# viswavi/speech-anonymization

Measured on AMD Instinct MI355X. Metric: audio frames/sec (node), ConvAE+gender-adv train step, higher is better.
Workload: dtype bf16x3; 1 GPU; ConvAE recon0.1+sex0.9 adversarial train step (L1 recon + NLL), shape M: 32 utt/GPU x 161120 samples (T=1008 frames), Fbank x2 + norm + fwd + bwd + clip + Adam + Noam; batch_per_gpu=32, frames_per_utt=1008, parallelism=dp1

## Files before the change

### include/sa_hip.h

```cpp
#ifndef SA_HIP_H
#define SA_HIP_H
#ifdef __cplusplus
extern "C" {
#endif

#define SA_F32 0
#define SA_BF16 1
#define SA_BF16X3 2
#define SA_BF16X1F 3
#define SA_FP8 4
#define SA_F64 5
#define SA_MAX_TAPS 5
#define SA_COMM_ID_BYTES 128

typedef struct SaTaps {
  int ntaps[2];
  int off[2][SA_MAX_TAPS];
  int widx[2][SA_MAX_TAPS];
} SaTaps;

typedef struct SaConvArgs {
  const void* x;
  const void* wp;
  const float* bias;
// ... 59 lines not shown
  const float* slabs; float* dst;
  int nslab, ntaps, cin, cout, sk, sn, st, accumulate, vec, pad_;
} SaWredDesc;
typedef struct SaWredMulti { int n, pad_; SaWredDesc d[SA_WRED_MAX]; } SaWredMulti;
int sa_wgrad_reduce_multi(const SaWredMulti* m, void* stream);

int sa_conv1toC(int dtype, const float* x, const float* w, const float* bias, void* y, int B, int L,
                int flip, float* stats, const void* ep_x, const float* ep_s1, const float* ep_t1,
                const float* ep_mean, const float* ep_rstd, void* stream);
int sa_conv1toC_ntiles(int L);
int sa_convCto1(int dtype, const void* x, const float* w, const float* bias, float* y, int B, int L,
                const float* s1, const float* t1, int swish, int flip, void* stream);
int sa_wgrad1C(int dtype, const float* u, const void* v, float* slabs, int B, int L, int chunk,
               int flip, const float* s1, const float* t1, int swish, void* stream);
int sa_wgrad1C_nchunk(int L, int chunk);
int sa_sum_slabs(const float* slabs, float* dst, int nslab, int n, int accumulate, void* stream);

typedef struct SaEwArgs {
  const void* g; const void* g2; const void* x; void* out;
  const float* s1; const float* t1;
  const float* mean; const float* rstd;
  const float* c1; const float* c2; const float* c3;
  int actbwd, xp_is_act, relu_mask, bstride;
  float* stats;
  int B, L, ntiles;
} SaEwArgs;

int sa_ew_stats(int dtype, int C, const SaEwArgs* a, void* stream);
int sa_ew_apply(int dtype, int C, const SaEwArgs* a, void* stream);
int sa_ew_ntiles(int L);
// ... 141 lines not shown
                  void* stream);
int sa_fc_wreduce(const float* wpart, int G, float* grads, void* stream);

int sa_cluster_mi(const float* X, const long long* y, const long long* idx, int iters, int n, int D,
                  int ncls, int k, float* mi, void* stream);

int sa_fbank(const float* wav, int B, int N, const float* window, const void* dft,
             const void* mel, float* feats, float* tilemax, void* stream);
int sa_fbank_table_elems(int which);
int sa_fbank_ntiles(int T);
int sa_fbank_scratch_bytes(int B);
int sa_fbank_normalize(const float* feats, const float* tilemax, int B, int T, int Tp,
                       const float* lens, float top_db, int batch_max, int update, int epoch,
                       int update_until_epoch, float* state, float* scratch, float* out,
                       void* stream);

int sa_add_layernorm_fwd(const void* x, const void* r, const void* gamma, const void* beta, void* y, void* s_out,
                         float* stat, int rows, int d, float eps, void* stream);
int sa_layernorm_bwd(const void* dy, const void* s, const float* stat, const void* gamma, void* ds, int rows,
                     int d, void* stream);
int sa_ln_leaky_fwd(const void* x, const void* gamma, const void* beta, void* y, float* stat, int rows, int d,
                    float eps, float slope, void* stream);
int sa_ln_leaky_bwd(const void* dy, const void* x, const float* stat, const void* gamma, const void* beta, void* dx,
                    int rows, int d, float slope, void* stream);
int sa_asr_block0_fwd(const void* x, const void* w, const void* bias, const void* gamma, const void* beta, void* y,
                      float* stat, int B, int T, int F, int C, float eps, float slope, void* stream);
int sa_asr_block0_bwd(const void* dy, const void* x, const void* w, const void* bias, const void* gamma,
                      const void* beta, const float* stat, float* part, void* dx, int B, int T, int F, int C,
                      float slope, void* stream);
int sa_reflect_pad_fwd(const void* x, void* y, int B, int T, int F, int C, void* stream);
// ... 16 lines not shown
```

### speech-anonymization_amd/_lib.py

```python
import ctypes as C
import os

import torch

_HERE = os.path.dirname(os.path.abspath(__file__))
LIB_PATH = os.environ.get("SA_HIP_LIB") or os.path.join(_HERE, "libsa_hip.so")

F32, BF16, BF16X3, BF16X1F, FP8, F64 = 0, 1, 2, 3, 4, 5
MAX_TAPS = 5

c_fp = C.POINTER(C.c_float)
vp = C.c_void_p


class SaTaps(C.Structure):
    _fields_ = [("ntaps", C.c_int * 2), ("off", (C.c_int * MAX_TAPS) * 2),
                ("widx", (C.c_int * MAX_TAPS) * 2)]


class SaConvArgs(C.Structure):
    _fields_ = [("x", vp), ("wp", vp), ("bias", vp), ("y", vp),
                ("s1", vp), ("t1", vp), ("s2", vp), ("t2", vp),
                ("swish", C.c_int), ("relu", C.c_int), ("stats", vp),
                ("B", C.c_int), ("Lin", C.c_int), ("Lout", C.c_int), ("ntiles", C.c_int),
# ... 67 lines not shown



class SaWredDesc(C.Structure):
    _fields_ = [("slabs", vp), ("dst", vp)] + [(k, C.c_int) for k in ("nslab", "ntaps", "cin", "cout", "sk", "sn", "st",
                                                                      "accumulate", "vec", "pad_")]


class SaWredMulti(C.Structure):
    _fields_ = [("n", C.c_int), ("pad_", C.c_int), ("d", SaWredDesc * WRED_MAX)]


SYMBOLS = [
    "sa_conv_gemm", "sa_abi_sizeof", "sa_conv_gemm_ntiles", "sa_conv_gemm_ntiles_tm", "sa_conv_gemm_set_tile_rows",
    "sa_conv_gemm_geometry", "sa_conv_gemm_set_impl", "sa_conv_gemm_route", "sa_conv_pp_set_tile_rows", "sa_pack_weights", "sa_pack_weights_multi", "sa_pack_scales_multi", "sa_wgrad", "sa_wgrad_kw", "sa_wgrad_reduce",
    "sa_conv1toC", "sa_conv1toC_ntiles", "sa_convCto1", "sa_wgrad1C", "sa_wgrad1C_nchunk",
    "sa_sum_slabs", "sa_ew_stats", "sa_ew_apply", "sa_ew_ntiles", "sa_act_stats",
    "sa_sum_partials", "sa_sum_rows_d", "sa_reduce_finalize", "sa_fin_in_fwd", "sa_fin_bn_fwd", "sa_fin_bn_eval", "sa_fin_norm_bwd", "sa_fin_bias",
    "sa_pool_fwd", "sa_pool_nseg", "sa_pool_gather", "sa_pool_fin", "sa_pool_bwd", "sa_dense", "sa_colsums",
    "sa_bn2d_bwd", "sa_dense_wgrad", "sa_log_softmax", "sa_log_softmax_bwd",
    "sa_loss_workspace_bytes", "sa_recon_loss", "sa_cls_losses", "sa_cosine_loss",
    "sa_tdnn_fwd", "sa_time_pool", "sa_leaky_affine", "sa_tdnn_bwd_input", "sa_tdnn_fold", "sa_time_pool_bwd",
    "sa_leaky_affine_bwd", "sa_cluster_mi", "sa_fbank", "sa_fbank_table_elems", "sa_fbank_ntiles", "sa_fbank_scratch_bytes", "sa_fbank_normalize",
    "sa_comm_unique_id", "sa_comm_init", "sa_comm_world", "sa_comm_allreduce", "sa_comm_allreduce_inline", "sa_comm_join", "sa_comm_ncalls",
    "sa_comm_destroy", "sa_head_fwd", "sa_head_bwd", "sa_head_max_rows",
    "sa_add_layernorm_fwd", "sa_layernorm_bwd", "sa_reflect_pad_fwd", "sa_reflect_pad_bwd", "sa_ln_leaky_fwd", "sa_ln_leaky_bwd", "sa_bias_multi", "sa_asr_block0_fwd", "sa_asr_block0_bwd", "sa_wgrad_reduce_multi", "sa_clip_grads",
    "sa_xv_tdnn_fwd_train", "sa_xv_tdnn_ntiles", "sa_xv_colsums", "sa_xv_tdnn_wgrad", "sa_xv_wgrad_reduce",
    "sa_xv_tdnn_dgrad", "sa_xv_pool_affine", "sa_xv_pool_affine_bwd",
    "sa_fc_tiles", "sa_fc_groups", "sa_fc_nparam", "sa_fc_nhead", "sa_fc_max_rows", "sa_fc_enc_fwd", "sa_fc_bn_fin",
    "sa_fc_mid_fwd", "sa_fc_head_fwd", "sa_fc_head_bwd", "sa_fc_mid_bwd", "sa_fc_bn_bwd_fin", "sa_fc_enc_bwd",
    "sa_fc_wreduce", "sa_fc_recon_fwd",
]

_lib = None


class SaHipError(RuntimeError):
    pass
# ... 60 lines not shown
```

### speech-anonymization_amd/brain.py

```python
import enum
import os
import types

import torch

from . import distributed as sdist


class Stage(enum.Enum):
    TRAIN = 1
    VALID = 2
    TEST = 3


class EpochCounter:

    def __init__(self, limit):
        self.current, self.limit = 0, int(limit)

    def __iter__(self):
        return self

    def __next__(self):
        if self.current < self.limit:
# ... 60 lines not shown

class Brain:
    GC_FREEZE_STEP = 8

    def __init__(self, modules=None, opt_class=None, hparams=None, run_opts=None, checkpointer=None):
        run_opts = dict(run_opts or {})
        self.device = torch.device(run_opts.get("device", "cuda:0" if torch.cuda.is_available() else "cpu"))
        if self.device.type == "cuda":
            torch.cuda.set_device(self.device)
        self.max_grad_norm = float(run_opts.get("max_grad_norm", 5.0))
        self.nonfinite_patience = int(run_opts.get("nonfinite_patience", 3))
        self.lazy_finite_check = bool(run_opts.get("lazy_finite_check", True))
        self.hip_graph = bool(run_opts.get("hip_graph", False)) and self.device.type == "cuda"
        self.gc_freeze = bool(run_opts.get("gc_freeze", True))
        self.fused_clip = bool(run_opts.get("fused_clip", os.environ.get("SA_FUSED_CLIP", "1") == "1"))
        self.distributed_launch = bool(run_opts.get("distributed_launch", sdist.is_distributed()))
        self.modules = torch.nn.ModuleDict(modules or {})
        self.dp_batch_sizes = run_opts.get("dp_batch_sizes", "equal")
        self.opt_class = opt_class
        self.hparams = types.SimpleNamespace(**(hparams or {}))
        self.checkpointer = checkpointer
        self.step, self.nonfinite_count, self.optimizer = 0, 0, None
        self.avg_train_loss = 0.0

    def compute_forward(self, batch, stage):
        raise NotImplementedError

    def compute_objectives(self, predictions, batch, stage):
        raise NotImplementedError

# ... 165 lines not shown
    def evaluate(self, test_set, max_key=None, min_key=None, **_):
        self.on_evaluate_start(max_key=max_key, min_key=min_key)
        self.on_stage_start(Stage.TEST, None)
        self.modules.eval()
        avg, n = 0.0, 0
        with torch.no_grad():
            for batch in test_set:
                n += 1
                avg += (float(self.evaluate_batch(batch, Stage.TEST)) - avg) / n
        self.on_stage_end(Stage.TEST, avg, None)
        return avg


class SexAnonymizationTraining(Brain):

    def features(self, wavs, wav_lens):
        feats = self.hparams.compute_features(wavs)
        current_epoch = self.hparams.epoch_counter.current
        pad = 36 if self.hparams.model_type != "fcae" else None
        return self.modules.normalize(feats, wav_lens, epoch=current_epoch, pad_multiple=pad)

    def compute_forward(self, batch, stage):
        batch = batch.to(self.device)
        wavs, wav_lens = batch.sig
        feats = self.features(wavs, wav_lens)
        return self.modules.ConvAE(feats)

    def compute_objectives(self, predictions, batch, stage):
        reconstructed_speech, sex_logits = predictions
        batch = batch.to(self.device)
        sex_label = batch.gender
        wavs, wav_lens = batch.sig
        feats = self.features(wavs, wav_lens)
        hp = self.hparams
        utility_loss = 0.0
        asr_brain = getattr(self, "asr_brain", None)
        if stage == Stage.TRAIN and hp.utility_loss_weight > 0 and asr_brain is not None:
            from . import asr
            tokens_bos, _ = batch.tokens_bos
            utility_loss = asr.utility_loss(asr_brain, hp.loss_utility, feats, reconstructed_speech,
# ... 65 lines not shown
    GRAPH_WARMUP = 3

    def _graph_key(self, batch):
        hp = self.hparams
        wavs, lens = batch.sig
        nrm = self.modules["normalize"] if "normalize" in self.modules else None
        upd = nrm is not None and hp.epoch_counter.current < getattr(nrm, "update_until_epoch", 0)
        st = self.optimizer.state if self.optimizer is not None else {}
        params = list(self.modules.ConvAE.parameters())
        tok = batch.tokens_bos[0]
        return (tuple(wavs.shape), str(wavs.dtype), hp.model_type, float(hp.recon_loss_weight),
                float(hp.sex_loss_weight), float(hp.utility_loss_weight),
                float(getattr(hp, "confusion_loss_weight", 0.0)), bool(upd),
                tuple(p.requires_grad for p in params),
                tuple(bool(st.get(p)) for p in params if not p.requires_grad),
                tuple(tok.shape), getattr(self, "asr_brain", None) is not None)

    def _step_core(self, batch):
        predictions = self.compute_forward(batch, Stage.TRAIN)
        loss = self.compute_objectives(predictions, batch, Stage.TRAIN)
        loss.backward()
        if getattr(self.hparams, "epoch_parity_schedule", False):
            self._zero_grads_of_frozen()
        self.check_gradients(loss)
        self.optimizer.step()
        return loss.detach()

    def _fit_batch_graph(self, batch):
        batch = batch.to(self.device)
        key = self._graph_key(batch)
        graphs = self.__dict__.setdefault("_graphs", {})
# ... 31 lines not shown
        ent["batch"].id = batch.id
        bad = self._poll_nonfinite()
        if bad:
            self.nonfinite_count += bad
            if self.nonfinite_count > self.nonfinite_patience:
                raise ValueError("Loss is not finite and patience is exhausted.")
        ent["graph"].replay()
        st = getattr(self, "_finite_state", None)
        if st is not None:
            st["event"].record()
            st["pending"] = True
        self.hparams.noam_annealing(self.optimizer)
        return ent["loss"]

    def fit_batch(self, batch):
        self.apply_epoch_schedule()
        if (self.hip_graph and self.hparams.gradient_accumulation == 1 and sdist.capturable()
                and self.optimizer is not None):
            return self._fit_batch_graph(batch)
        predictions = self.compute_forward(batch, Stage.TRAIN)
        loss = self.compute_objectives(predictions, batch, Stage.TRAIN)
        (loss / self.hparams.gradient_accumulation).backward()
        if self.step % self.hparams.gradient_accumulation == 0:
            if getattr(self.hparams, "epoch_parity_schedule", False):
                self._zero_grads_of_frozen()
            self.check_gradients(loss)
            self.optimizer.step()
            self.optimizer.zero_grad()
            self.hparams.noam_annealing(self.optimizer)
        return loss.detach()

    def evaluate_batch(self, batch, stage):
        with torch.no_grad():
            predictions = self.compute_forward(batch, stage=stage)
# ... 82 lines not shown
```

### speech-anonymization_amd/convae.py

```python
import functools
import os

import torch
import torch.nn as nn

from . import distributed as sdist
from . import ops
from . import _lib as L
from ._lib import SaHipError

K5 = 5
CONVT_WG_TAPS = [(1, 0), (1, 1), (0, 0), (0, 1), (-1, 0)]


class _ParamOnly(nn.Module):

    def forward(self, x):
        raise SaHipError("parameter container only; use ConvAutoencoder.forward")


class GLU(_ParamOnly):
    pass


# ... 49 lines not shown
        self.sex_classifier = TDNNSexClassifier(2)
        self.act_dtype, self.kcode = ops.PRECISIONS[precision]
        self.dec_kcode = self.kcode
        self.dgrad_kcode = ops.DGRAD_CODE[precision]
        self.cache_wgrad_operand = cache_wgrad_operand
        self.fuse_apply = True
        self.overlap_wgrad = os.environ.get("SA_OVERLAP_WGRAD", "0") == "1"
        self.pooling_noise = pooling_noise
        self.sync_bn = sync_bn
        self.fused_finalize = os.environ.get("SA_FUSED_FINALIZE", "0") == "1"
        self.fused_in_fwd = os.environ.get("SA_FUSED_IN_FWD", "0") == "1"
        self.overlap_head = os.environ.get("SA_OVERLAP_HEAD", "0") == "1"
        self.fused_head = os.environ.get("SA_FUSED_HEAD", "1") == "1"
        self.batch_bias = os.environ.get("SA_BATCH_BIAS", "1") == "1"
        self.batch_wred = os.environ.get("SA_BATCH_WRED", "1") == "1"
        self.dp_batch_sizes = None
        self.bwd_reload_bf16 = os.environ.get("SA_BWD_RELOAD_BF16", "0") == "1"
        self.store_bf16_probe = int(os.environ.get("SA_STORE_BF16_PROBE", "0"))

    def forward(self, feats):
        names, params = self._named_params()
        return _ConvAEFn.apply(self, names, feats, *params)

    def _named_params(self):
        c = self.__dict__.get("_np_cache")
        if c is None or any(o[n] is not p for o, n, p in c[2]):
            names, params, owners = [], [], []
            for mname, mod in self.named_modules():
                for pname, p in mod._parameters.items():
                    if p is not None:
# ... 602 lines not shown
            xp4 = (n4[2], n4[3])
            g, st = cg(g, pw(t + "0.weight", "conv_dgrad"), None, 128, 128, 1, 1,
                       ops.taps_conv_dgrad_s1(5, 1, 0), L4, want_stats=True, ep=bn_ep(y4, bn_n, xp4))
            da = bn_finish(g, st, y4, bn_n, L4, "sex_classifier.norm", None, 0, xp=xp4)
            side_join()
            flush_bias()
            if need_stage["sex_classifier"]:
                buckets.reduce_stage("sex_classifier")
            return da

        def decoder_bwd():
            d_rec = torch.zeros(B, T, 80, device=dev) if recon_unused else d_recon
            g_rec = d_rec.reshape(B, Ltot).contiguous().float()
            if need["decoder.8.bias"]:
                setg("decoder.8.bias", ops.sum_partials(g_rec.view(4 * B, Ltot // 4), 1, n=Ltot // 4).sum())
            if need["decoder.8.weight"]:
                G["decoder.8.weight"] = ops.wgrad1C(g_rec, y8, newg("decoder.8.weight"), flip=True,
                                                    s1=n8[2], t1=n8[3], swish=True)
            g, st = ops.conv1toC(g_rec, P["decoder.8.weight"], None, dt, flip=True, want_stats=True,
                                 ep=dict(x=y8, s1=n8[2], t1=n8[3], mean=n8[0], rstd=n8[1]))
            if model.store_bf16_probe >= 2:
                _round_first(g)
            in_decoder[0] = True
            g = in_finish(g, st, y8, n8, 32, Ltot, "decoder.6", "decoder.5.bias")
            convT_wgrad("decoder.5.weight", y7, g, 64, 32, L2)
            g, st = cg(g, pw("decoder.5.weight", "convT_dgrad"), None, 32, 64, 2, 1,
                       ops.taps_convT_dgrad(), L2, want_stats=True)
            bias_from(st, "decoder.4.bias", 64)
            conv_wgrad("decoder.4.weight", y6, g, 64, 64, 1, L2, K5, 1, 2, s1=n6[2], t1=n6[3], swish=True)
            g, st = cg(g, pw("decoder.4.weight", "conv_dgrad"), None, 64, 64, 1, 1,
                       ops.taps_conv_dgrad_s1(K5, 1, 2), L2, want_stats=True, ep=in_ep(y6, n6))
            g = in_finish(g, st, y6, n6, 64, L2, "decoder.2", "decoder.1.bias")
            convT_wgrad("decoder.1.weight", y5, g, 128, 64, L4)
            g, st = cg(g, pw("decoder.1.weight", "convT_dgrad"), None, 64, 128, 2, 1,
                       ops.taps_convT_dgrad(), L4, want_stats=True)
# ... 58 lines not shown
```

### speech-anonymization_amd/csrc/sa_fbank.hip

```cpp
#include "sa_common.h"

#define SA_NFFT 400
#define SA_HOP 160
#define SA_NBIN 201
#define SA_FK 208
#define SA_FKS 13
#define SA_BINT 7
#define SA_MELT 3
#define SA_NMEL 80
#define SA_FB_FRAMES 32

__device__ static inline void sa_split3(float v, bf16_t& h, bf16_t& m, bf16_t& l) {
  h = (bf16_t)v;
  const float r1 = v - (float)h;
  m = (bf16_t)r1;
  l = (bf16_t)(r1 - (float)m);
}

__global__ __launch_bounds__(256) void sa_fbank_kernel(const float* __restrict__ wav, int N, int T,
                                                       const float* __restrict__ window,
                                                       const bf16x8* __restrict__ dft,
                                                       const bf16x8* __restrict__ mel,
                                                       float* __restrict__ feats,
                                                       float* __restrict__ tilemax, int ntiles) {
// ... 264 lines not shown
  if (!feats || !tilemax || !lens || !state || !scratch || !out || B <= 0 || T <= 0 || Tp < T)
    return -22;
  hipStream_t st = reinterpret_cast<hipStream_t>(stream);
  float* fl = scratch;
  double* part = reinterpret_cast<double*>(scratch + ((B + 1) & ~1));
  hipLaunchKernelGGL(sa_fbank_utt_partial_kernel, dim3(SA_UTT_CHUNKS, B), dim3(256), 0, st, feats,
                     tilemax, sa_div_up(T, SA_FB_FRAMES), B, T, lens, top_db, batch_max, fl, part);
  hipLaunchKernelGGL(sa_norm_update_kernel, dim3(1), dim3(640), 0, st, part, lens, B, T, update, epoch,
                     update_until_epoch, state);
  const size_t n4 = (size_t)Tp * SA_NMEL / 4;
  hipLaunchKernelGGL(sa_norm_apply_kernel, dim3((unsigned)((n4 + 255) / 256), B), dim3(256), 0, st,
                     feats, fl, state, T, Tp, out);
  hipError_t e = hipGetLastError();
  return e == hipSuccess ? 0 : -(int)e;
}
```

### speech-anonymization_amd/csrc/sa_small.hip

```cpp
#include "sa_common.h"

#define SA_K15 15
#define SA_C32 32

template <typename T>
__global__ __launch_bounds__(256) void sa_conv1toC_kernel(const float* __restrict__ x,
                                                          const float* __restrict__ w,
                                                          const float* __restrict__ bias,
                                                          T* __restrict__ y, int L, int flip,
                                                          float* __restrict__ stats, int ntiles,
                                                          const T* __restrict__ ep_x,
                                                          const float* __restrict__ ep_s1,
                                                          const float* __restrict__ ep_t1,
                                                          const float* __restrict__ ep_mean,
                                                          const float* __restrict__ ep_rstd) {
  constexpr int VEC = Tr<T>::VEC, CH = SA_C32 / VEC, PPP = 256 / CH, TILE = 512;
  __shared__ float xs[TILE + SA_K15 - 1];
  __shared__ __attribute__((aligned(16))) float ws[SA_K15][SA_C32];
  __shared__ float red[PPP][SA_C32][2];
  const int tid = threadIdx.x, b = blockIdx.y, l0 = blockIdx.x * TILE;
  for (int i = tid; i < TILE + SA_K15 - 1; i += 256) {
    const int g = l0 + i - 7;
    xs[i] = (g >= 0 && g < L) ? x[(size_t)b * L + g] : 0.0f;
  }
// ... 261 lines not shown
                          int chunk, int flip, const float* s1, const float* t1, int swish,
                          void* stream) {
  if (!u || !v || !slabs || B <= 0 || L <= 0 || chunk <= 0 || chunk % 256) return -22;
  hipStream_t st = reinterpret_cast<hipStream_t>(stream);
  dim3 grid(sa_div_up(L, chunk), B);
  if (dtype == SA_BF16)
    hipLaunchKernelGGL(sa_wgrad1C_kernel<bf16_t>, grid, dim3(256), 0, st, u,
                       reinterpret_cast<const bf16_t*>(v), slabs, L, chunk, flip, s1, t1, swish);
  else
    hipLaunchKernelGGL(sa_wgrad1C_kernel<float>, grid, dim3(256), 0, st, u,
                       reinterpret_cast<const float*>(v), slabs, L, chunk, flip, s1, t1, swish);
  hipError_t e = hipGetLastError();
  return e == hipSuccess ? 0 : -(int)e;
}

__global__ __launch_bounds__(256) void sa_sum_slabs_kernel(const float* __restrict__ slabs,
                                                           float* __restrict__ dst, int nslab, int n,
                                                           int accumulate) {
  __shared__ double part[16][17];
  const int o = threadIdx.x & 15, q = threadIdx.x >> 4, i = blockIdx.x * 16 + o;
  double s = 0.0;
  if (i < n) {
#pragma unroll 4
    for (int k = q; k < nslab; k += 16) s += (double)slabs[(size_t)k * n + i];
  }
  part[q][o] = s;
  __syncthreads();
  if (q == 0 && i < n) {
    double t = 0.0;
#pragma unroll
// ... 14 lines not shown
```

### speech-anonymization_amd/endtoend.py

```python
import functools

import torch
import torch.nn as nn

from . import _lib as L
from . import ops
from ._lib import SaHipError
from .convae import GLU, CONVT_WG_TAPS, K5
from .xvector import EncoderClassifier


class ConvReconstruction(nn.Module):
    def __init__(self, sex_classifier=None, precision="bf16x3"):
        super().__init__()
        if precision not in ("bf16x3", "f32"):
            raise SaHipError("ConvReconstruction runs in precision bf16x3 or f32")
        self.precision = precision
        self.act_dtype, self.kcode = ops.PRECISIONS[precision]
        self.encoder = nn.Sequential(
            nn.Conv1d(1, 32, 15, 1, 7), nn.InstanceNorm1d(32, affine=True), GLU(),
            nn.Conv1d(32, 64, 5, 2, 2), nn.InstanceNorm1d(64, affine=True), GLU(),
            nn.Conv1d(64, 64, 5, 1, 2), nn.InstanceNorm1d(64, affine=True), GLU(),
            nn.ConvTranspose1d(64, 32, 5, 2, 2, output_padding=1), nn.InstanceNorm1d(32, affine=True), GLU(),
            nn.Conv1d(32, 1, 15, 1, 7),
        )
        self.sex_classifier = sex_classifier if sex_classifier is not None else EncoderClassifier()
        for p in self.sex_classifier.parameters():
            p.requires_grad = False
        self.sex_classifier.eval()

    def train(self, mode=True):
        super().train(mode)
        self.sex_classifier.eval()
# ... 91 lines not shown
            dg, db = newg(prefix + ".weight"), newg(prefix + ".bias")
            c1, c2, c3 = ops.fin_norm_bwd(sums, sums, B * C, C, Ln, P[prefix + ".weight"], nrm[0], nrm[1],
                                          dgamma=dg, dbeta=db)
            G[prefix + ".weight"], G[prefix + ".bias"] = dg, db
            st2 = ops.ew("apply", g, y, C, out=g, c1=c1, c2=c2, c3=c3)
            if need[bias_key]:
                G[bias_key] = ops.fin_bias(ops.sum_partials(st2, B), B, C, newg(bias_key))
            return g

        def in_ep(y, nrm):
            return dict(mode=1, x=y, s1=nrm[2], t1=nrm[3], mean=nrm[0], rstd=nrm[1])

        g_rec = d_recon.reshape(B, Ltot).contiguous().float()
        if need["encoder.12.bias"]:
            G["encoder.12.bias"] = ops.sum_partials(g_rec.view(4 * B, Ltot // 4), 1, n=Ltot // 4).sum().float().reshape(1)
        if need["encoder.12.weight"]:
            G["encoder.12.weight"] = ops.wgrad1C(g_rec, y3, newg("encoder.12.weight"), flip=True,
                                                 s1=n3[2], t1=n3[3], swish=True)
        g, st = ops.conv1toC(g_rec, P["encoder.12.weight"], None, dt, flip=True, want_stats=True,
                             ep=dict(x=y3, s1=n3[2], t1=n3[3], mean=n3[0], rstd=n3[1]))
        g = norm_bwd(g, st, y3, n3, 32, Ltot, "encoder.10", "encoder.9.bias")
        if need["encoder.9.weight"]:
            G["encoder.9.weight"] = wg(y2, g, 64, 32, 1, 2, CONVT_WG_TAPS, L2, newg("encoder.9.weight"),
                                       (32 * K5, K5, 1), s1=n2[2], t1=n2[3], swish=True)
        g, st = ops.conv_gemm(g, pack("encoder.9.weight", "convT_dgrad"), None, 32, 64, 2, 1,
                              ops.taps_convT_dgrad(), L2, want_stats=True, ep=in_ep(y2, n2), code=code)
        g = norm_bwd(g, st, y2, n2, 64, L2, "encoder.7", "encoder.6.bias")
        taps5 = [(k - 2, 0) for k in range(K5)]
        if need["encoder.6.weight"]:
            G["encoder.6.weight"] = wg(y1, g, 64, 64, 1, 1, taps5, L2, newg("encoder.6.weight"),
                                       (K5, 64 * K5, 1), s1=n1[2], t1=n1[3], swish=True)
        g, st = ops.conv_gemm(g, pack("encoder.6.weight", "conv_dgrad"), None, 64, 64, 1, 1,
                              ops.taps_conv_dgrad_s1(K5, 1, 2), L2, want_stats=True, ep=in_ep(y1, n1),
                              code=code)
        g = norm_bwd(g, st, y1, n1, 64, L2, "encoder.4", "encoder.3.bias")
# ... 14 lines not shown
```

### speech-anonymization_amd/features.py

```python
import ctypes as C
import math

import numpy as np
import torch

from . import _lib as L

N_FFT, HOP, NBIN, FK, KSTEPS, BIN_TILES, MEL_ROWS, MEL_COLS = 400, 160, 201, 208, 13, 7, 208, 96


def _hamming(n):
    i = np.arange(n, dtype=np.float64)
    return (0.54 - 0.46 * np.cos(2.0 * np.pi * i / n)).astype(np.float32)


def _split_bf16(v, planes):
    out, r = [], v.float()
    for _ in range(planes):
        h = r.to(torch.bfloat16)
        out.append(h)
        r = r - h.float()
    return out


# ... 76 lines not shown
        tmax = torch.empty(B, lib.sa_fbank_ntiles(T), dtype=torch.float32, device=wav.device)
        L.check(lib.sa_fbank(L.ptr(wav), B, N, L.ptr(self.window), L.ptr(self.dft), L.ptr(self.mel),
                             L.ptr(raw), L.ptr(tmax), L.stream()), "sa_fbank")
        return FbankFeatures(raw, tmax, self.top_db, self.batch_max)


class InputNormalization(torch.nn.Module):

    def __init__(self, norm_type="global", update_until_epoch=3, pad_multiple=None):
        super().__init__()
        if norm_type != "global":
            raise L.SaHipError("only norm_type='global' is implemented (convae.yaml:269-271)")
        self.update_until_epoch = update_until_epoch
        self.pad_multiple = pad_multiple
        self.register_buffer("state", torch.zeros(161), persistent=False)

    @property
    def count(self):
        return int(self.state[0].item())

    @property
    def glob_mean(self):
        return self.state[1:81]

    @property
    def glob_std(self):
        return self.state[81:161]

    @torch.no_grad()
    def forward(self, feats, lengths, epoch=0, pad_multiple=None):
        lib = L.load()
        if isinstance(feats, FbankFeatures):
            raw, tmax, top_db, bmax = feats.raw, feats.tilemax, feats.top_db, feats.batch_max
        else:
            raw = feats.contiguous().float()
            B, T, _ = raw.shape
            tmax = torch.full((B, lib.sa_fbank_ntiles(T)), -1e30, device=raw.device)
            top_db, bmax = 0.0, False
        B, T, _ = raw.shape
        if self.state.device != raw.device:
            self.to(raw.device)
        m = pad_multiple if pad_multiple is not None else self.pad_multiple
        Tp = T if not m or T % m == 0 else T + (m - T % m)
        lens = lengths.to(device=raw.device, dtype=torch.float32).contiguous()
        out = torch.empty(B, Tp, 80, dtype=torch.float32, device=raw.device)
        scratch = torch.empty(lib.sa_fbank_scratch_bytes(B) // 4, dtype=torch.float32, device=raw.device)
        L.check(lib.sa_fbank_normalize(L.ptr(raw), L.ptr(tmax), B, T, Tp, L.ptr(lens),
                                       C.c_float(top_db), int(bmax), int(self.training), int(epoch),
                                       int(self.update_until_epoch), L.ptr(self.state),
                                       L.ptr(scratch), L.ptr(out), L.stream()), "sa_fbank_normalize")
        return out

    def state_dict(self, *a, **k):
        return {"count": self.count, "glob_mean": self.glob_mean.clone(),
                "glob_std": self.glob_std.clone(), "spk_dict_mean": {}, "spk_dict_std": {},
                "spk_dict_count": {}}

    def load_state_dict(self, sd, strict=True):
        with torch.no_grad():
            self.state[0] = float(sd["count"])
            self.state[1:81] = sd["glob_mean"].to(self.state.device).float()
            self.state[81:161] = sd["glob_std"].to(self.state.device).float()
```

### speech-anonymization_amd/ops.py

```python
import ctypes as C
import functools

import torch

from . import _lib as L

UP2 = [[(1, 0), (0, 2), (-1, 4)], [(1, 1), (0, 3)]]


def taps_conv(K, dil, pad):
    return [[(k * dil - pad, k) for k in range(K)]]


def taps_conv_dgrad_s1(K, dil, pad):
    return [[(pad - k * dil, k) for k in range(K)]]


def taps_convT_dgrad(K=5, pad=2):
    return [[(k - pad, k) for k in range(K)]]


def _f(t):
    return L.ptr(t)

# ... 265 lines not shown
    return y


def wgrad1C(u, v, dst, flip=False, s1=None, t1=None, swish=False, accumulate=False, chunk=2048):
    lib = L.load()
    B, Ln = u.shape
    nch = lib.sa_wgrad1C_nchunk(Ln, chunk)
    slabs = torch.empty(B * nch, 32 * 15, dtype=torch.float32, device=u.device)
    L.check(lib.sa_wgrad1C(L.dt_code(v.dtype), _f(u), _f(v), _f(slabs), B, Ln, chunk, int(flip),
                           _f(s1), _f(t1), int(swish), L.stream()), "sa_wgrad1C")
    L.check(lib.sa_sum_slabs(_f(slabs), _f(dst), B * nch, 32 * 15, int(accumulate), L.stream()),
            "sa_sum_slabs")
    return dst


def sum_partials(part, nbatch, n=None, rows=False):
    lib = L.load()
    if n is None:
        n = part.shape[-2] * part.shape[-1]
    total = part.numel()
    nslab = total // (nbatch * n)
    if nbatch == 1 and nslab >= 512 and part.dim() == 4 and part.shape[0] > 1:
        R = part.shape[0]
        mid = torch.empty(R, n, dtype=torch.float64, device=part.device)
        L.check(lib.sa_sum_partials(_f(part), _f(mid), R, nslab // R, n, L.stream()), "sa_sum_partials")
        if rows:
            return mid
        out = torch.empty(1, n, dtype=torch.float64, device=part.device)
        L.check(lib.sa_sum_rows_d(_f(mid), _f(out), R, n, L.stream()), "sa_sum_rows_d")
        return out
# ... 380 lines not shown
```

Measured before the change: 3.828 million frames/s.

## Fuse 1-to-C conv backward dgrad+wgrad and compute normalized features once per step

Adds a fused sa_bwd1C kernel that computes the data gradient, its instance-norm stats and the weight-gradient slabs of the final 32-to-1 conv in one pass. This replaces the separate wgrad1C and conv1toC launches and avoids rereading the gradient and activation twice. Adds a paired fbank normalization that computes the input and the target features from one fbank pass, which drops the second feature computation per training step. It replays the running-mean update twice so the statistics keep the same semantics. The risks are cache-key invalidation based on tensor pointer and version, and more complex normalization state handling.

```diff
diff --git a/include/sa_hip.h b/include/sa_hip.h
--- a/include/sa_hip.h
+++ b/include/sa_hip.h
@@ -97,6 +97,9 @@
 int sa_wgrad1C(int dtype, const float* u, const void* v, float* slabs, int B, int L, int chunk,
                int flip, const float* s1, const float* t1, int swish, void* stream);
 int sa_wgrad1C_nchunk(int L, int chunk);
+int sa_bwd1C(int dtype, const float* u, const void* v, const float* w, void* g, float* stats, float* slabs,
+             int B, int L, int chunk, int flip, const float* s1, const float* t1, const float* mean,
+             const float* rstd, void* stream);
 int sa_sum_slabs(const float* slabs, float* dst, int nslab, int n, int accumulate, void* stream);
 
 typedef struct SaEwArgs {
@@ -268,6 +271,10 @@
                        const float* lens, float top_db, int batch_max, int update, int epoch,
                        int update_until_epoch, float* state, float* scratch, float* out,
                        void* stream);
+int sa_fbank_normalize_pair(const float* feats, const float* tilemax, int B, int T, int Tp,
+                            const float* lens, float top_db, int batch_max, int update, int epoch,
+                            int update_until_epoch, float* state, float* scratch, float* snap,
+                            float* out1, float* out2, void* stream);
 
 int sa_add_layernorm_fwd(const void* x, const void* r, const void* gamma, const void* beta, void* y, void* s_out,
                          float* stat, int rows, int d, float eps, void* stream);
diff --git a/speech-anonymization_amd/_lib.py b/speech-anonymization_amd/_lib.py
--- a/speech-anonymization_amd/_lib.py
+++ b/speech-anonymization_amd/_lib.py
@@ -105,14 +105,14 @@
 SYMBOLS = [
     "sa_conv_gemm", "sa_abi_sizeof", "sa_conv_gemm_ntiles", "sa_conv_gemm_ntiles_tm", "sa_conv_gemm_set_tile_rows",
     "sa_conv_gemm_geometry", "sa_conv_gemm_set_impl", "sa_conv_gemm_route", "sa_conv_pp_set_tile_rows", "sa_pack_weights", "sa_pack_weights_multi", "sa_pack_scales_multi", "sa_wgrad", "sa_wgrad_kw", "sa_wgrad_reduce",
-    "sa_conv1toC", "sa_conv1toC_ntiles", "sa_convCto1", "sa_wgrad1C", "sa_wgrad1C_nchunk",
+    "sa_conv1toC", "sa_conv1toC_ntiles", "sa_convCto1", "sa_wgrad1C", "sa_wgrad1C_nchunk", "sa_bwd1C",
     "sa_sum_slabs", "sa_ew_stats", "sa_ew_apply", "sa_ew_ntiles", "sa_act_stats",
     "sa_sum_partials", "sa_sum_rows_d", "sa_reduce_finalize", "sa_fin_in_fwd", "sa_fin_bn_fwd", "sa_fin_bn_eval", "sa_fin_norm_bwd", "sa_fin_bias",
     "sa_pool_fwd", "sa_pool_nseg", "sa_pool_gather", "sa_pool_fin", "sa_pool_bwd", "sa_dense", "sa_colsums",
     "sa_bn2d_bwd", "sa_dense_wgrad", "sa_log_softmax", "sa_log_softmax_bwd",
     "sa_loss_workspace_bytes", "sa_recon_loss", "sa_cls_losses", "sa_cosine_loss",
     "sa_tdnn_fwd", "sa_time_pool", "sa_leaky_affine", "sa_tdnn_bwd_input", "sa_tdnn_fold", "sa_time_pool_bwd",
-    "sa_leaky_affine_bwd", "sa_cluster_mi", "sa_fbank", "sa_fbank_table_elems", "sa_fbank_ntiles", "sa_fbank_scratch_bytes", "sa_fbank_normalize",
+    "sa_leaky_affine_bwd", "sa_cluster_mi", "sa_fbank", "sa_fbank_table_elems", "sa_fbank_ntiles", "sa_fbank_scratch_bytes", "sa_fbank_normalize", "sa_fbank_normalize_pair",
     "sa_comm_unique_id", "sa_comm_init", "sa_comm_world", "sa_comm_allreduce", "sa_comm_allreduce_inline", "sa_comm_join", "sa_comm_ncalls",
     "sa_comm_destroy", "sa_head_fwd", "sa_head_bwd", "sa_head_max_rows",
     "sa_add_layernorm_fwd", "sa_layernorm_bwd", "sa_reflect_pad_fwd", "sa_reflect_pad_bwd", "sa_ln_leaky_fwd", "sa_ln_leaky_bwd", "sa_bias_multi", "sa_asr_block0_fwd", "sa_asr_block0_bwd", "sa_wgrad_reduce_multi", "sa_clip_grads",
diff --git a/speech-anonymization_amd/brain.py b/speech-anonymization_amd/brain.py
--- a/speech-anonymization_amd/brain.py
+++ b/speech-anonymization_amd/brain.py
@@ -98,6 +98,7 @@
         self.hip_graph = bool(run_opts.get("hip_graph", False)) and self.device.type == "cuda"
         self.gc_freeze = bool(run_opts.get("gc_freeze", True))
         self.fused_clip = bool(run_opts.get("fused_clip", os.environ.get("SA_FUSED_CLIP", "1") == "1"))
+        self.front_end_once = bool(run_opts.get("front_end_once", os.environ.get("SA_FRONT_END_ONCE", "1") == "1"))
         self.distributed_launch = bool(run_opts.get("distributed_launch", sdist.is_distributed()))
         self.modules = torch.nn.ModuleDict(modules or {})
         self.dp_batch_sizes = run_opts.get("dp_batch_sizes", "equal")
@@ -293,16 +294,35 @@
 
 class SexAnonymizationTraining(Brain):
 
+    @staticmethod
+    def _sig_key(wavs, wav_lens):
+        return tuple((t.data_ptr(), tuple(t.shape), t.dtype, t._version) for t in (wavs, wav_lens))
+
     def features(self, wavs, wav_lens):
+        stash, self._target_stash = self.__dict__.get("_target_stash"), None
+        if stash is not None and stash[0] == self._sig_key(wavs, wav_lens):
+            return stash[1]
         feats = self.hparams.compute_features(wavs)
         current_epoch = self.hparams.epoch_counter.current
         pad = 36 if self.hparams.model_type != "fcae" else None
         return self.modules.normalize(feats, wav_lens, epoch=current_epoch, pad_multiple=pad)
 
+    def _features_pair(self, wavs, wav_lens):
+        feats = self.hparams.compute_features(wavs)
+        pad = 36 if self.hparams.model_type != "fcae" else None
+        inp, target = self.modules.normalize.forward_pair(feats, wav_lens, epoch=self.hparams.epoch_counter.current,
+                                                          pad_multiple=pad)
+        self._target_stash = (self._sig_key(wavs, wav_lens), target)
+        return inp
+
     def compute_forward(self, batch, stage):
         batch = batch.to(self.device)
         wavs, wav_lens = batch.sig
-        feats = self.features(wavs, wav_lens)
+        if (stage == Stage.TRAIN and self.__dict__.get("_in_fit_batch") and self.front_end_once
+                and hasattr(self.modules.normalize, "forward_pair")):
+            feats = self._features_pair(wavs, wav_lens)
+        else:
+            feats = self.features(wavs, wav_lens)
         return self.modules.ConvAE(feats)
 
     def compute_objectives(self, predictions, batch, stage):
@@ -398,7 +418,8 @@
                 float(getattr(hp, "confusion_loss_weight", 0.0)), bool(upd),
                 tuple(p.requires_grad for p in params),
                 tuple(bool(st.get(p)) for p in params if not p.requires_grad),
-                tuple(tok.shape), getattr(self, "asr_brain", None) is not None)
+                tuple(tok.shape), getattr(self, "asr_brain", None) is not None,
+                self.front_end_once, bool(not upd and getattr(nrm, "_count_positive", False)))
 
     def _step_core(self, batch):
         predictions = self.compute_forward(batch, Stage.TRAIN)
@@ -460,10 +481,19 @@
         return ent["loss"]
 
     def fit_batch(self, batch):
+        self._target_stash, self._in_fit_batch = None, True
+        try:
+            return self._fit_batch(batch)
+        finally:
+            self._target_stash, self._in_fit_batch = None, False
+
+    def _fit_batch(self, batch):
         self.apply_epoch_schedule()
         if (self.hip_graph and self.hparams.gradient_accumulation == 1 and sdist.capturable()
                 and self.optimizer is not None):
             return self._fit_batch_graph(batch)
+        if self.front_end_once:
+            batch = batch.to(self.device)
         predictions = self.compute_forward(batch, Stage.TRAIN)
         loss = self.compute_objectives(predictions, batch, Stage.TRAIN)
         (loss / self.hparams.gradient_accumulation).backward()
diff --git a/speech-anonymization_amd/convae.py b/speech-anonymization_amd/convae.py
--- a/speech-anonymization_amd/convae.py
+++ b/speech-anonymization_amd/convae.py
@@ -87,6 +87,7 @@
         self.fused_head = os.environ.get("SA_FUSED_HEAD", "1") == "1"
         self.batch_bias = os.environ.get("SA_BATCH_BIAS", "1") == "1"
         self.batch_wred = os.environ.get("SA_BATCH_WRED", "1") == "1"
+        self.fused_bwd1c = os.environ.get("SA_FUSED_BWD1C", "1") == "1"
         self.dp_batch_sizes = None
         self.bwd_reload_bf16 = os.environ.get("SA_BWD_RELOAD_BF16", "0") == "1"
         self.store_bf16_probe = int(os.environ.get("SA_STORE_BF16_PROBE", "0"))
@@ -719,11 +720,15 @@
             g_rec = d_rec.reshape(B, Ltot).contiguous().float()
             if need["decoder.8.bias"]:
                 setg("decoder.8.bias", ops.sum_partials(g_rec.view(4 * B, Ltot // 4), 1, n=Ltot // 4).sum())
-            if need["decoder.8.weight"]:
-                G["decoder.8.weight"] = ops.wgrad1C(g_rec, y8, newg("decoder.8.weight"), flip=True,
-                                                    s1=n8[2], t1=n8[3], swish=True)
-            g, st = ops.conv1toC(g_rec, P["decoder.8.weight"], None, dt, flip=True, want_stats=True,
-                                 ep=dict(x=y8, s1=n8[2], t1=n8[3], mean=n8[0], rstd=n8[1]))
+            if need["decoder.8.weight"] and model.fused_bwd1c:
+                g, st, G["decoder.8.weight"] = ops.bwd1C(g_rec, y8, P["decoder.8.weight"], newg("decoder.8.weight"),
+                                                         n8[2], n8[3], n8[0], n8[1])
+            else:
+                if need["decoder.8.weight"]:
+                    G["decoder.8.weight"] = ops.wgrad1C(g_rec, y8, newg("decoder.8.weight"), flip=True,
+                                                        s1=n8[2], t1=n8[3], swish=True)
+                g, st = ops.conv1toC(g_rec, P["decoder.8.weight"], None, dt, flip=True, want_stats=True,
+                                     ep=dict(x=y8, s1=n8[2], t1=n8[3], mean=n8[0], rstd=n8[1]))
             if model.store_bf16_probe >= 2:
                 _round_first(g)
             in_decoder[0] = True
diff --git a/speech-anonymization_amd/csrc/sa_fbank.hip b/speech-anonymization_amd/csrc/sa_fbank.hip
--- a/speech-anonymization_amd/csrc/sa_fbank.hip
+++ b/speech-anonymization_amd/csrc/sa_fbank.hip
@@ -302,3 +302,109 @@
   hipError_t e = hipGetLastError();
   return e == hipSuccess ? 0 : -(int)e;
 }
+
+
+__device__ static inline float sa_running_avg(float w, float old, float cur) {
+#pragma clang fp contract(off)
+  const float t = (1.0f - w) * old;
+  return fmaf(w, cur, t);
+}
+
+__global__ __launch_bounds__(640) void sa_norm_update2_kernel(const double* __restrict__ part,
+                                                              const float* __restrict__ lens, int B, int T,
+                                                              int update, int epoch, int update_until_epoch,
+                                                              float* state, float* __restrict__ snap) {
+  __shared__ float lm[8][SA_NMEL], ls[8][SA_NMEL];
+  const int f = threadIdx.x % SA_NMEL, q = threadIdx.x / SA_NMEL;
+  const float count = state[0];
+  float cm = 0.f, cs = 0.f;
+  for (int b = q; b < B; b += 8) {
+    int n = (int)rintf(lens[b] * (float)T);
+    if (n > T) n = T;
+    double s = 0.0, sq = 0.0;
+#pragma unroll
+    for (int c = 0; c < SA_UTT_CHUNKS; ++c) {
+      const double* d = part + (((size_t)b * SA_UTT_CHUNKS + c) * SA_NMEL + f) * 2;
+      s += d[0]; sq += d[1];
+    }
+    const double m = s / n;
+    double var = n > 1 ? (sq - s * m) / (n - 1) : 0.0;
+    if (var < 0.0) var = 0.0;
+    cm += (float)m;
+    cs += fmaxf((float)sqrt(var), 1e-10f);
+  }
+  lm[q][f] = cm; ls[q][f] = cs;
+  __syncthreads();
+  if (q == 0) {
+    cm = 0.f; cs = 0.f;
+#pragma unroll
+    for (int r = 0; r < 8; ++r) { cm += lm[r][f]; cs += ls[r][f]; }
+    cm /= B; cs /= B;
+    float gm = state[1 + f], gs = state[1 + SA_NMEL + f], cnt = count;
+#pragma unroll
+    for (int rep = 0; rep < 2; ++rep) {
+      if (update) {
+        if (cnt == 0.0f) { gm = cm; gs = cs; }
+        else if (epoch < update_until_epoch) {
+          const float w = 1.0f / (cnt + 1.0f);
+          gm = sa_running_avg(w, gm, cm);
+          gs = sa_running_avg(w, gs, cs);
+        }
+        cnt = cnt + 1.0f;
+      }
+      if (rep == 0) { snap[f] = gm; snap[SA_NMEL + f] = gs; }
+    }
+    if (update) { state[1 + f] = gm; state[1 + SA_NMEL + f] = gs; }
+  }
+  __syncthreads();
+  if (threadIdx.x == 0 && update) state[0] = (count + 1.0f) + 1.0f;
+}
+
+__global__ void sa_norm_apply2_kernel(const float* __restrict__ feats, const float* __restrict__ floor_b,
+                                      const float* __restrict__ st1, const float* __restrict__ st2, int T,
+                                      int Tp, float* __restrict__ out1, float* __restrict__ out2) {
+  const int b = blockIdx.y;
+  const size_t i = (size_t)blockIdx.x * blockDim.x + threadIdx.x;
+  if (i >= (size_t)Tp * SA_NMEL / 4) return;
+  const size_t e = i * 4;
+  const int t = (int)(e / SA_NMEL), f = (int)(e % SA_NMEL);
+  float4 o1 = make_float4(0.f, 0.f, 0.f, 0.f), o2 = o1;
+  if (t < T) {
+    const float4 x = *reinterpret_cast<const float4*>(feats + ((size_t)b * T) * SA_NMEL + e);
+    const float fl = floor_b[b];
+    const float c0 = fmaxf(x.x, fl), c1 = fmaxf(x.y, fl), c2 = fmaxf(x.z, fl), c3 = fmaxf(x.w, fl);
+    const float* gm = st1 + f;
+    const float* gs = st1 + SA_NMEL + f;
+    o1.x = (c0 - gm[0]) / gs[0]; o1.y = (c1 - gm[1]) / gs[1];
+    o1.z = (c2 - gm[2]) / gs[2]; o1.w = (c3 - gm[3]) / gs[3];
+    gm = st2 + f; gs = st2 + SA_NMEL + f;
+    o2.x = (c0 - gm[0]) / gs[0]; o2.y = (c1 - gm[1]) / gs[1];
+    o2.z = (c2 - gm[2]) / gs[2]; o2.w = (c3 - gm[3]) / gs[3];
+  }
+  *reinterpret_cast<float4*>(out1 + ((size_t)b * Tp) * SA_NMEL + e) = o1;
+  *reinterpret_cast<float4*>(out2 + ((size_t)b * Tp) * SA_NMEL + e) = o2;
+}
+
+extern "C" int sa_fbank_normalize_pair(const float* feats, const float* tilemax, int B, int T, int Tp,
+                                       const float* lens, float top_db, int batch_max, int update,
+                                       int epoch, int update_until_epoch, float* state, float* scratch,
+                                       float* snap, float* out1, float* out2, void* stream) {
+  if (!feats || !tilemax || !lens || !state || !scratch || !snap || !out1 || B <= 0 || T <= 0 || Tp < T)
+    return -22;
+  hipStream_t st = reinterpret_cast<hipStream_t>(stream);
+  float* fl = scratch;
+  double* part = reinterpret_cast<double*>(scratch + ((B + 1) & ~1));
+  hipLaunchKernelGGL(sa_fbank_utt_partial_kernel, dim3(SA_UTT_CHUNKS, B), dim3(256), 0, st, feats,
+                     tilemax, sa_div_up(T, SA_FB_FRAMES), B, T, lens, top_db, batch_max, fl, part);
+  hipLaunchKernelGGL(sa_norm_update2_kernel, dim3(1), dim3(640), 0, st, part, lens, B, T, update, epoch,
+                     update_until_epoch, state, snap);
+  const size_t n4 = (size_t)Tp * SA_NMEL / 4;
+  const dim3 grid((unsigned)((n4 + 255) / 256), B);
+  if (out2)
+    hipLaunchKernelGGL(sa_norm_apply2_kernel, grid, dim3(256), 0, st, feats, fl, snap, state + 1, T, Tp,
+                       out1, out2);
+  else
+    hipLaunchKernelGGL(sa_norm_apply_kernel, grid, dim3(256), 0, st, feats, fl, state, T, Tp, out1);
+  hipError_t e = hipGetLastError();
+  return e == hipSuccess ? 0 : -(int)e;
+}
diff --git a/speech-anonymization_amd/csrc/sa_small.hip b/speech-anonymization_amd/csrc/sa_small.hip
--- a/speech-anonymization_amd/csrc/sa_small.hip
+++ b/speech-anonymization_amd/csrc/sa_small.hip
@@ -299,6 +299,171 @@
   return e == hipSuccess ? 0 : -(int)e;
 }
 
+template <typename T>
+__global__ __launch_bounds__(256, Tr<T>::VEC == 4 ? 3 : 2) void sa_bwd1C_kernel(const float* __restrict__ u,
+                                                       const T* __restrict__ v,
+                                                       const float* __restrict__ w,
+                                                       T* __restrict__ gout, float* __restrict__ stats,
+                                                       int ntiles, float* __restrict__ slabs, int L,
+                                                       int chunk, int flip,
+                                                       const float* __restrict__ s1,
+                                                       const float* __restrict__ t1,
+                                                       const float* __restrict__ mean,
+                                                       const float* __restrict__ rstd) {
+  constexpr int VEC = Tr<T>::VEC, CH = SA_C32 / VEC, RPP = 256 / CH, TILE = 256, PITCH = 33;
+  __shared__ float us[TILE + SA_K15 - 1 + 1];
+  __shared__ float vs[TILE * PITCH];
+  __shared__ __attribute__((aligned(16))) float ws[SA_K15][SA_C32];
+  __shared__ float red[RPP][SA_C32][2];
+  __shared__ __attribute__((aligned(16))) float pv[4][SA_C32];
+  const int tid = threadIdx.x, lane = tid & 63, wave = tid >> 6, b = blockIdx.y;
+  const int lbeg = blockIdx.x * chunk;
+  int lend = lbeg + chunk; if (lend > L) lend = L;
+  const int c = tid % CH, r0 = tid / CH;
+  float ssum[VEC], ssq[VEC];
+#pragma unroll
+  for (int j = 0; j < VEC; ++j) { ssum[j] = 0.f; ssq[j] = 0.f; }
+  if (tid < 4 * SA_C32) {
+    const float* src = tid < 32 ? s1 : tid < 64 ? t1 : tid < 96 ? mean : rstd;
+    pv[tid >> 5][tid & 31] = src[(size_t)b * SA_C32 + (tid & 31)];
+  }
+  for (int i = tid; i < SA_K15 * SA_C32; i += 256) {
+    const int k = i / SA_C32, cc = i % SA_C32;
+    ws[k][cc] = w[cc * SA_K15 + (flip ? SA_K15 - 1 - k : k)];
+  }
+  const int m = lane & 15, j4 = lane >> 4;
+  const bool mval = m < SA_K15;
+  const int kk = mval ? (flip ? SA_K15 - 1 - m : m) : 0;
+  const int qa = wave * 64 + 16 * j4;
+  f32x4 acc0 = {0.f, 0.f, 0.f, 0.f}, acc1 = {0.f, 0.f, 0.f, 0.f};
+  constexpr int NIT = TILE / RPP, NU = (TILE + SA_K15 - 1 + 255) / 256;
+  uint4 raw[NIT];
+  float rawu[NU];
+  auto issue_v = [&](int l0, int i) {
+    const int g = l0 + r0 + i * RPP;
+    raw[i] = make_uint4(0, 0, 0, 0);
+    if (g < lend) raw[i] = *reinterpret_cast<const uint4*>(v + ((size_t)b * L + g) * SA_C32 + c * VEC);
+  };
+  auto issue_u = [&](int l0) {
+#pragma unroll
+    for (int i = 0; i < NU; ++i) {
+      const int g = l0 + tid + i * 256 - 7;
+      rawu[i] = (l0 < lend && tid + i * 256 < TILE + SA_K15 - 1 && g >= 0 && g < L) ? u[(size_t)b * L + g] : 0.0f;
+    }
+  };
+#pragma unroll
+  for (int i = 0; i < NIT; ++i) issue_v(lbeg, i);
+  issue_u(lbeg);
+  __syncthreads();
+  for (int l0 = lbeg; l0 < lend; l0 += TILE) {
+#pragma unroll
+    for (int i = 0; i < NU; ++i)
+      if (tid + i * 256 < TILE + SA_K15 - 1) us[tid + i * 256] = rawu[i];
+#pragma unroll
+    for (int i = 0; i < NIT; ++i) {
+      const int r = r0 + i * RPP, g = l0 + r;
+      float f[VEC];
+      Tr<T>::unpack(raw[i], f);
+      if (g < lend) {
+        int z0 = c * VEC; asm volatile("" : "+v"(z0));
+#pragma unroll
+        for (int j = 0; j < VEC; ++j) f[j] = sa_swish(fmaf(f[j], pv[0][z0 + j], pv[1][z0 + j]));
+      }
+#pragma unroll
+      for (int j = 0; j < VEC; ++j) vs[r * PITCH + c * VEC + j] = f[j];
+    }
+    __syncthreads();
+    issue_u(l0 + TILE);
+#pragma unroll
+    for (int i = 0; i < NIT; ++i) {
+      const int r = r0 + i * RPP, g = l0 + r;
+      float xv[VEC];
+      Tr<T>::unpack(raw[i], xv);
+      issue_v(l0 + TILE, i);
+      if (g < lend) {
+#pragma clang fp contract(off)
+        float acc[VEC], xn[VEC];
+#pragma unroll
+        for (int j = 0; j < VEC; ++j) acc[j] = 0.0f;
+#pragma unroll
+        for (int k = 0; k < SA_K15; ++k) {
+          const float uv = us[r + k];
+#pragma unroll
+          for (int j = 0; j < VEC; ++j) acc[j] = fmaf(uv, ws[k][c * VEC + j], acc[j]);
+        }
+        int z0 = c * VEC; asm volatile("" : "+v"(z0));
+#pragma unroll
+        for (int j = 0; j < VEC; ++j) {
+          acc[j] *= sa_swish_grad(fmaf(xv[j], pv[0][z0 + j], pv[1][z0 + j]));
+          xn[j] = (xv[j] - pv[2][z0 + j]) * pv[3][z0 + j];
+        }
+        const uint4 o = Tr<T>::pack(acc);
+        *reinterpret_cast<uint4*>(gout + ((size_t)b * L + g) * SA_C32 + c * VEC) = o;
+        float f[VEC];
+        Tr<T>::unpack(o, f);
+#pragma unroll
+        for (int j = 0; j < VEC; ++j) { ssum[j] += f[j]; ssq[j] = fmaf(f[j], xn[j], ssq[j]); }
+      }
+    }
+    const bool flush = (((l0 - lbeg) / TILE) & 1) || l0 + TILE >= lend;
+    if (flush) {
+#pragma unroll
+      for (int j = 0; j < VEC; ++j) {
+        red[r0][c * VEC + j][0] = ssum[j]; red[r0][c * VEC + j][1] = ssq[j];
+        ssum[j] = 0.f; ssq[j] = 0.f;
+      }
+    }
+#pragma unroll 4
+    for (int t = 0; t < 16; ++t) {
+      const int q = qa + t;
+      const float av = mval ? us[q + kk] : 0.0f;
+      const float b0 = vs[q * PITCH + m], b1 = vs[q * PITCH + 16 + m];
+      acc0 = __builtin_amdgcn_mfma_f32_16x16x4f32(av, b0, acc0, 0, 0, 0);
+      acc1 = __builtin_amdgcn_mfma_f32_16x16x4f32(av, b1, acc1, 0, 0, 0);
+    }
+    __syncthreads();
+    if (flush && tid < SA_C32) {
+      float s = 0.f, q = 0.f;
+      for (int r = 0; r < RPP; ++r) { s += red[r][tid][0]; q += red[r][tid][1]; }
+      float* d = stats + (((size_t)b * ntiles + l0 / 512) * SA_C32 + tid) * 2;
+      d[0] = s; d[1] = q;
+    }
+  }
+  float* part = vs;
+#pragma unroll
+  for (int i = 0; i < 4; ++i) {
+    part[(wave * 16 + 4 * j4 + i) * 32 + m] = acc0[i];
+    part[(wave * 16 + 4 * j4 + i) * 32 + 16 + m] = acc1[i];
+  }
+  __syncthreads();
+  for (int o = tid; o < SA_K15 * SA_C32; o += 256) {
+    const int k = o / SA_C32, cc = o % SA_C32;
+    const float sum = ((part[(0 * 16 + k) * 32 + cc] + part[(1 * 16 + k) * 32 + cc]) +
+                       part[(2 * 16 + k) * 32 + cc]) + part[(3 * 16 + k) * 32 + cc];
+    slabs[((size_t)b * gridDim.x + blockIdx.x) * (SA_C32 * SA_K15) + cc * SA_K15 + k] = sum;
+  }
+}
+
+extern "C" int sa_bwd1C(int dtype, const float* u, const void* v, const float* w, void* g, float* stats,
+                        float* slabs, int B, int L, int chunk, int flip, const float* s1,
+                        const float* t1, const float* mean, const float* rstd, void* stream) {
+  if (!u || !v || !w || !g || !stats || !slabs || B <= 0 || L <= 0 || chunk <= 0 || chunk % 512) return -22;
+  if (!s1 || !t1 || !mean || !rstd) return -22;
+  hipStream_t st = reinterpret_cast<hipStream_t>(stream);
+  const int nt = sa_div_up(L, 512);
+  dim3 grid(sa_div_up(L, chunk), B);
+  if (dtype == SA_BF16)
+    hipLaunchKernelGGL(sa_bwd1C_kernel<bf16_t>, grid, dim3(256), 0, st, u,
+                       reinterpret_cast<const bf16_t*>(v), w, reinterpret_cast<bf16_t*>(g), stats, nt,
+                       slabs, L, chunk, flip, s1, t1, mean, rstd);
+  else
+    hipLaunchKernelGGL(sa_bwd1C_kernel<float>, grid, dim3(256), 0, st, u,
+                       reinterpret_cast<const float*>(v), w, reinterpret_cast<float*>(g), stats, nt,
+                       slabs, L, chunk, flip, s1, t1, mean, rstd);
+  hipError_t e = hipGetLastError();
+  return e == hipSuccess ? 0 : -(int)e;
+}
+
 __global__ __launch_bounds__(256) void sa_sum_slabs_kernel(const float* __restrict__ slabs,
                                                            float* __restrict__ dst, int nslab, int n,
                                                            int accumulate) {
diff --git a/speech-anonymization_amd/endtoend.py b/speech-anonymization_amd/endtoend.py
--- a/speech-anonymization_amd/endtoend.py
+++ b/speech-anonymization_amd/endtoend.py
@@ -1,4 +1,5 @@
 import functools
+import os
 
 import torch
 import torch.nn as nn
@@ -17,6 +18,7 @@
             raise SaHipError("ConvReconstruction runs in precision bf16x3 or f32")
         self.precision = precision
         self.act_dtype, self.kcode = ops.PRECISIONS[precision]
+        self.fused_bwd1c = os.environ.get("SA_FUSED_BWD1C", "1") == "1"
         self.encoder = nn.Sequential(
             nn.Conv1d(1, 32, 15, 1, 7), nn.InstanceNorm1d(32, affine=True), GLU(),
             nn.Conv1d(32, 64, 5, 2, 2), nn.InstanceNorm1d(64, affine=True), GLU(),
@@ -138,11 +140,15 @@
         g_rec = d_recon.reshape(B, Ltot).contiguous().float()
         if need["encoder.12.bias"]:
             G["encoder.12.bias"] = ops.sum_partials(g_rec.view(4 * B, Ltot // 4), 1, n=Ltot // 4).sum().float().reshape(1)
-        if need["encoder.12.weight"]:
-            G["encoder.12.weight"] = ops.wgrad1C(g_rec, y3, newg("encoder.12.weight"), flip=True,
-                                                 s1=n3[2], t1=n3[3], swish=True)
-        g, st = ops.conv1toC(g_rec, P["encoder.12.weight"], None, dt, flip=True, want_stats=True,
-                             ep=dict(x=y3, s1=n3[2], t1=n3[3], mean=n3[0], rstd=n3[1]))
+        if need["encoder.12.weight"] and model.fused_bwd1c:
+            g, st, G["encoder.12.weight"] = ops.bwd1C(g_rec, y3, P["encoder.12.weight"], newg("encoder.12.weight"),
+                                                      n3[2], n3[3], n3[0], n3[1])
+        else:
+            if need["encoder.12.weight"]:
+                G["encoder.12.weight"] = ops.wgrad1C(g_rec, y3, newg("encoder.12.weight"), flip=True,
+                                                     s1=n3[2], t1=n3[3], swish=True)
+            g, st = ops.conv1toC(g_rec, P["encoder.12.weight"], None, dt, flip=True, want_stats=True,
+                                 ep=dict(x=y3, s1=n3[2], t1=n3[3], mean=n3[0], rstd=n3[1]))
         g = norm_bwd(g, st, y3, n3, 32, Ltot, "encoder.10", "encoder.9.bias")
         if need["encoder.9.weight"]:
             G["encoder.9.weight"] = wg(y2, g, 64, 32, 1, 2, CONVT_WG_TAPS, L2, newg("encoder.9.weight"),
diff --git a/speech-anonymization_amd/features.py b/speech-anonymization_amd/features.py
--- a/speech-anonymization_amd/features.py
+++ b/speech-anonymization_amd/features.py
@@ -114,6 +114,7 @@
         self.update_until_epoch = update_until_epoch
         self.pad_multiple = pad_multiple
         self.register_buffer("state", torch.zeros(161), persistent=False)
+        self._count_positive = False
 
     @property
     def count(self):
@@ -127,8 +128,7 @@
     def glob_std(self):
         return self.state[81:161]
 
-    @torch.no_grad()
-    def forward(self, feats, lengths, epoch=0, pad_multiple=None):
+    def _prepare(self, feats, lengths, pad_multiple):
         lib = L.load()
         if isinstance(feats, FbankFeatures):
             raw, tmax, top_db, bmax = feats.raw, feats.tilemax, feats.top_db, feats.batch_max
@@ -143,13 +143,39 @@
         m = pad_multiple if pad_multiple is not None else self.pad_multiple
         Tp = T if not m or T % m == 0 else T + (m - T % m)
         lens = lengths.to(device=raw.device, dtype=torch.float32).contiguous()
+        scratch = torch.empty(lib.sa_fbank_scratch_bytes(B) // 4, dtype=torch.float32, device=raw.device)
+        return raw, tmax, top_db, bmax, B, T, Tp, lens, scratch
+
+    @torch.no_grad()
+    def forward(self, feats, lengths, epoch=0, pad_multiple=None):
+        lib = L.load()
+        raw, tmax, top_db, bmax, B, T, Tp, lens, scratch = self._prepare(feats, lengths, pad_multiple)
         out = torch.empty(B, Tp, 80, dtype=torch.float32, device=raw.device)
-        scratch = torch.empty(lib.sa_fbank_scratch_bytes(B) // 4, dtype=torch.float32, device=raw.device)
         L.check(lib.sa_fbank_normalize(L.ptr(raw), L.ptr(tmax), B, T, Tp, L.ptr(lens),
                                        C.c_float(top_db), int(bmax), int(self.training), int(epoch),
                                        int(self.update_until_epoch), L.ptr(self.state),
                                        L.ptr(scratch), L.ptr(out), L.stream()), "sa_fbank_normalize")
+        if self.training:
+            self._count_positive = True
         return out
+
+    @torch.no_grad()
+    def forward_pair(self, feats, lengths, epoch=0, pad_multiple=None):
+        lib = L.load()
+        raw, tmax, top_db, bmax, B, T, Tp, lens, scratch = self._prepare(feats, lengths, pad_multiple)
+        same = (not self.training) or (int(epoch) >= int(self.update_until_epoch) and self._count_positive)
+        out1 = torch.empty(B, Tp, 80, dtype=torch.float32, device=raw.device)
+        out2 = out1 if same else torch.empty_like(out1)
+        snap = torch.empty(160, dtype=torch.float32, device=raw.device)
+        L.check(lib.sa_fbank_normalize_pair(L.ptr(raw), L.ptr(tmax), B, T, Tp, L.ptr(lens),
+                                            C.c_float(top_db), int(bmax), int(self.training), int(epoch),
+                                            int(self.update_until_epoch), L.ptr(self.state),
+                                            L.ptr(scratch), L.ptr(snap), L.ptr(out1),
+                                            None if same else L.ptr(out2), L.stream()),
+                "sa_fbank_normalize_pair")
+        if self.training:
+            self._count_positive = True
+        return out1, out2
 
     def state_dict(self, *a, **k):
         return {"count": self.count, "glob_mean": self.glob_mean.clone(),
@@ -159,5 +185,6 @@
     def load_state_dict(self, sd, strict=True):
         with torch.no_grad():
             self.state[0] = float(sd["count"])
+            self._count_positive = float(sd["count"]) > 0
             self.state[1:81] = sd["glob_mean"].to(self.state.device).float()
             self.state[81:161] = sd["glob_std"].to(self.state.device).float()
diff --git a/speech-anonymization_amd/ops.py b/speech-anonymization_amd/ops.py
--- a/speech-anonymization_amd/ops.py
+++ b/speech-anonymization_amd/ops.py
@@ -303,6 +303,20 @@
     return dst
 
 
+def bwd1C(u, v, w, dst, s1, t1, mean, rstd, flip=True, accumulate=False, chunk=2048):
+    lib = L.load()
+    B, Ln = u.shape
+    nch = lib.sa_wgrad1C_nchunk(Ln, chunk)
+    g = torch.empty(B, Ln, 32, dtype=v.dtype, device=u.device)
+    stats = torch.empty(B, lib.sa_conv1toC_ntiles(Ln), 32, 2, dtype=torch.float32, device=u.device)
+    slabs = torch.empty(B * nch, 32 * 15, dtype=torch.float32, device=u.device)
+    L.check(lib.sa_bwd1C(L.dt_code(v.dtype), _f(u), _f(v), _f(w), _f(g), _f(stats), _f(slabs), B, Ln, chunk,
+                         int(flip), _f(s1), _f(t1), _f(mean), _f(rstd), L.stream()), "sa_bwd1C")
+    L.check(lib.sa_sum_slabs(_f(slabs), _f(dst), B * nch, 32 * 15, int(accumulate), L.stream()),
+            "sa_sum_slabs")
+    return g, stats, dst
+
+
 def sum_partials(part, nbatch, n=None, rows=False):
     lib = L.load()
     if n is None:
```

New measurement: 3.912 million frames/s (median of 6 runs). 2.2% higher.
